# fauzanardh/OsuFusion

Measured on AMD Instinct MI355X. Metric: denoise-steps/sec (train fwd+bwd) at B=32 L=4096, higher is better.
Workload: dtype bf16; 1 GPU; full OsuFusion UNet dim_h=256 (343.5M params) train step: fwd+bwd+grad-norm+clip+AdamW, per-GPU batch 32, L=4096, x (B,6,L), audio (B,96,L) [BASELINE 'audio-ctx=1024x128' maps to the (B,1024,L/8) bottleneck code]; global_batch=32, seq_len=4096, parallelism=dp1

## Files before the change

osufusion_amd/csrc/gemm.hip:

```cpp
#include "common.hpp"
#include <optional>
#include <stdlib.h>

struct RowMap {
  int Lin, Lout, stride, pad, mode;
};
__device__ __forceinline__ int map_row(const RowMap& rm, int i, int t) {
  if (rm.mode == 3) {
    if (t == 3) return (i == rm.Lout - 2) ? rm.Lin - 1 : -1;
    int e = i - t;
    if (e < 0 || (e & 1)) return -1;
    e >>= 1;
    return e < rm.Lin ? e : -1;
  }
  int s = i * rm.stride + t - rm.pad;
  if (rm.mode == 2) {
    if (s < 0 || s >= 2 * rm.Lin) return -1;
    return s >> 1;
  }
  if (rm.mode == 1 && s == rm.Lin) s = rm.Lin - 2;
  return (s >= 0 && s < rm.Lin) ? s : -1;
}

struct GemmArgs {
// ... 1282 lines not shown
          typedef __attribute__((ext_vector_type(8))) short s16x8;
          s16x8 va = {lo[0][0], lo[0][1], lo[0][2], lo[0][3], lo[1][0], lo[1][1], lo[1][2], lo[1][3]};
          s16x8 vb = {hi[0][0], hi[0][1], hi[0][2], hi[0][3], hi[1][0], hi[1][1], hi[1][2], hi[1][3]};
          fa[i] = __builtin_bit_cast(bf16x8, va);
          fb[i] = __builtin_bit_cast(bf16x8, vb);
        }
#pragma unroll
        for (int i = 0; i < 2; ++i)
#pragma unroll
          for (int j = 0; j < 2; ++j)
            acc[i][j] = __builtin_amdgcn_mfma_f32_32x32x16_bf16(fa[i], fb[j], acc[i][j], 0, 0, 0);
      }
    } else if constexpr (SPLIT) {
#pragma unroll
      for (int kk = 0; kk < 2; ++kk) {
        bf16x8 ah[2], al[2], bh[2], bl[2];
#pragma unroll
        for (int i = 0; i < 2; ++i) {
          float xa[8], xb[8];
#pragma unroll
          for (int e = 0; e < 8; ++e) {
            const int row = 16 * kk + 8 * lh + e;
            xa[e] = *reinterpret_cast<const float*>(sy + row * ROWB + (wr * 64 + i * 32 + lr) * 4);
            xb[e] = *reinterpret_cast<const float*>(sx + row * ROWB + (wc * 64 + i * 32 + lr) * 4);
          }
          split_bf16x8(xa, ah[i], al[i]);
          split_bf16x8(xb, bh[i], bl[i]);
        }
#pragma unroll
        for (int i = 0; i < 2; ++i)
#pragma unroll
          for (int j = 0; j < 2; ++j) mfma_x3(acc[i][j], ah[i], al[i], bh[j], bl[j]);
      }
    } else {
#pragma unroll 4
      for (int ks = 0; ks < 16; ++ks) {
        const int row = 2 * ks + lh;
        float fa[2], fb[2];
#pragma unroll
        for (int i = 0; i < 2; ++i) {
          fa[i] = *reinterpret_cast<const float*>(sy + row * ROWB + (wr * 64 + i * 32 + lr) * 4);
          fb[i] = *reinterpret_cast<const float*>(sx + row * ROWB + (wc * 64 + i * 32 + lr) * 4);
        }
#pragma unroll
        for (int i = 0; i < 2; ++i)
#pragma unroll
          for (int j = 0; j < 2; ++j) acc[i][j] = __builtin_amdgcn_mfma_f32_32x32x2f32(fa[i], fb[j], acc[i][j], 0, 0, 0);
      }
    }
  };

  load_regs(m_begin, ry0, rx0);
  if (m_begin + BKM < m_end) load_regs(m_begin + BKM, ry1, rx1);
  store_lds(0, ry0, rx0);
  __syncthreads();
  for (int mb = m_begin; mb < m_end; mb += 2 * BKM) {
    if (mb + 2 * BKM < m_end) load_regs(mb + 2 * BKM, ry0, rx0);
    compute(0);
    if (mb + BKM < m_end) store_lds(1, ry1, rx1);
    __syncthreads();
    if (mb + BKM >= m_end) break;
    if (mb + 3 * BKM < m_end) load_regs(mb + 3 * BKM, ry1, rx1);
    compute(1);
    if (mb + 2 * BKM < m_end) store_lds(0, ry0, rx0);
    __syncthreads();
  }

  float* dW = g.dW + (long)t * g.tapstride;
#pragma unroll
  for (int i = 0; i < 2; ++i)
#pragma unroll
    for (int j = 0; j < 2; ++j) {
      int n2 = n2_0 + wc * 64 + j * 32 + lr;
      if (n2 < g.N2) {
#pragma unroll
        for (int r = 0; r < 16; ++r) {
          int n1 = n1_0 + wr * 64 + i * 32 + (r & 3) + 8 * (r >> 2) + 4 * lh;
          if (n1 < g.N1) atomic_add_f32(dW + (long)n1 * g.ldw + (long)n2 * g.es, acc[i][j][r]);
        }
      }
    }
}

template <bool IL = false>
__device__ __forceinline__ void tn_big_store(const WgradArgs& g, const f32x16 (&acc)[4][2], int split, int t, int n1_0, int n2_0, int wr, int wc,
                                             int lr, int lh) {
  auto n1_of = [&](int i, int r) {
    const int rho = (r & 3) + 8 * (r >> 2) + 4 * lh;
    return n1_0 + wr * 128 + (IL ? 4 * rho + i : i * 32 + rho);
  };
  if (g.ws && g.ws_pk && !IL) {
    uint32_t* out = reinterpret_cast<uint32_t*>(g.ws) + ((long)split * g.taps + t) * (g.N1 >> 1) * g.N2;
#pragma unroll
    for (int i = 0; i < 4; ++i)
#pragma unroll
      for (int j = 0; j < 2; ++j) {
        const int n2 = n2_0 + wc * 64 + j * 32 + lr;
        if (n2 < g.N2) {
#pragma unroll
          for (int r = 0; r < 16; r += 2) {
            const int n1 = n1_of(i, r);
            if (n1 < g.N1) out[(long)(n1 >> 1) * g.N2 + n2] = pack_bf16x2(acc[i][j][r], acc[i][j][r + 1]);
          }
        }
      }
    return;
  }
  if (g.ws) {
    float* out = g.ws + ((long)split * g.taps + t) * g.N1 * g.N2;
#pragma unroll
    for (int i = 0; i < 4; ++i)
#pragma unroll
      for (int j = 0; j < 2; ++j) {
        const int n2 = n2_0 + wc * 64 + j * 32 + lr;
        if (n2 < g.N2) {
#pragma unroll
          for (int r = 0; r < 16; ++r) {
            const int n1 = n1_of(i, r);
            if (n1 < g.N1) out[(long)n1 * g.N2 + n2] = acc[i][j][r];
          }
        }
      }
    return;
  }
  float* dW = g.dW + (long)t * g.tapstride;
#pragma unroll
  for (int i = 0; i < 4; ++i)
#pragma unroll
    for (int j = 0; j < 2; ++j) {
      const int n2 = n2_0 + wc * 64 + j * 32 + lr;
      if (n2 < g.N2) {
#pragma unroll
        for (int r = 0; r < 16; ++r) {
          const int n1 = n1_of(i, r);
          if (n1 < g.N1) atomic_add_f32(dW + (long)n1 * g.ldw + (long)n2 * g.es, acc[i][j][r]);
        }
      }
    }
}

__device__ __forceinline__ float bf16x2_sum(unsigned w, float acc) {
  typedef __attribute__((ext_vector_type(2))) __bf16 bf2;
  return __builtin_amdgcn_fdot2_f32_bf16(__builtin_bit_cast(bf2, w), __builtin_bit_cast(bf2, 0x3F803F80u), acc, false);
}
__device__ __forceinline__ float bf16x8_sum(u32x2 lo, u32x2 hi, float acc) {
  const unsigned w0 = lo.x, w1 = lo.y, w2 = hi.x, w3 = hi.y;
  return bf16x2_sum(w3, bf16x2_sum(w2, bf16x2_sum(w1, bf16x2_sum(w0, acc))));
}

#define OSUF_TR_READ(dst, addr, off) asm volatile("ds_read_b64_tr_b16 %0, %1 offset:%2" : "=v"(dst) : "v"(addr), "n"(off))

__global__ __launch_bounds__(512, 2) void gemm_tn_big_kernel(WgradArgs g) {
  extern __shared__ __attribute__((aligned(16))) char smem[];
  constexpr int BKM = 64, ROWB = 512, TILEB = BKM * ROWB;
  const int tid = threadIdx.x, lane = tid & 63;
  const int wave = __builtin_amdgcn_readfirstlane(tid >> 6);
  const int wr = wave >> 2, wc = wave & 3;
  const int tiles_n2 = (g.N2 + kBig - 1) / kBig;
  const int tiles_n1 = (g.N1 + kBig - 1) / kBig;
  const int ntile = tiles_n1 * tiles_n2;
  const int xcd = blockIdx.x & 7, qid = blockIdx.x >> 3;
  const int unit = xcd * (((int)gridDim.x >> 3) / g.taps) + qid / g.taps;
  const int t = qid % g.taps;
  const int split = unit / ntile, tile = unit % ntile;
  const int n1_0 = (tile / tiles_n2) * kBig, n2_0 = (tile % tiles_n2) * kBig;
  const int m_begin = split * g.rows_per_split;
  const int m_end = min(g.M, m_begin + g.rows_per_split);
  if (m_begin >= m_end) return;
  const bf16_t* dY = reinterpret_cast<const bf16_t*>(g.dY);
  const bf16_t* X = reinterpret_cast<const bf16_t*>(g.X);
  const char* zero = reinterpret_cast<const char*>(g_zero_page);

  int srow[4], scol[4];
#pragma unroll
  for (int i = 0; i < 4; ++i) {
    srow[i] = (wave * 4 + i) * 2 + (lane >> 5);
    scol[i] = ((lane & 31) ^ ((srow[i] & 3) << 2)) * 8;
  }
  int sb_[4], sp_[4];
  const char* py[4];
  bool y_ok[4], x_ok[4];
#pragma unroll
  for (int i = 0; i < 4; ++i) {
    const int m = m_begin + srow[i];
    sb_[i] = m / g.rm.Lout;
    sp_[i] = m - sb_[i] * g.rm.Lout;
    y_ok[i] = n1_0 + scol[i] < g.N1;
    x_ok[i] = n2_0 + scol[i] < g.N2;
    py[i] = reinterpret_cast<const char*>(dY + (long)m * g.ldy + n1_0 + scol[i]);
  }
  const long ystep = (long)BKM * g.ldy * (long)sizeof(bf16_t);
  auto issue = [&](int mb, int buf) {
    char* sy = smem + buf * 2 * TILEB + wave * 4096;
    char* sx = sy + TILEB;
#pragma unroll
    for (int i = 0; i < 4; ++i) {
      const bool in = mb + srow[i] < m_end;
      const char* qy = (in && y_ok[i]) ? py[i] : zero;
      const char* qx = zero;
      if (in && x_ok[i]) {
        const int s2 = map_row(g.rm, sp_[i], t);
        if (s2 >= 0) qx = reinterpret_cast<const char*>(X + (long)(sb_[i] * g.rm.Lin + s2) * g.ldx + n2_0 + scol[i]);
      }
      __builtin_amdgcn_global_load_lds((gas_ptr)qy, (las_ptr)(sy + i * 1024), 16, 0, 0);
      __builtin_amdgcn_global_load_lds((gas_ptr)qx, (las_ptr)(sx + i * 1024), 16, 0, 0);
      py[i] += ystep;
      sp_[i] += BKM;
      while (sp_[i] >= g.rm.Lout) { sp_[i] -= g.rm.Lout; ++sb_[i]; }
    }
  };

  f32x16 acc[4][2];
#pragma unroll
  for (int i = 0; i < 4; ++i)
#pragma unroll
    for (int j = 0; j < 2; ++j)
#pragma unroll
      for (int r = 0; r < 16; ++r) acc[i][j][r] = 0.f;

  const int lr = lane & 31, lh = lane >> 5;
  const int ip = lane & 15, cb = ((lane >> 4) & 1) * 16, tq = ip >> 2, tp = ip & 3;
  uint32_t offA[4], offB[2];
  const uint32_t lds0 = (uint32_t)(uintptr_t)(LDS_PTR(char))smem;
#pragma unroll
  for (int i = 0; i < 4; ++i) offA[i] = (8 * lh + tq) * ROWB + ((((wr * 128 + i * 32 + cb + 4 * tp) * 2)) ^ (tq << 6));
#pragma unroll
  for (int j = 0; j < 2; ++j) offB[j] = TILEB + (8 * lh + tq) * ROWB + ((((wc * 64 + j * 32 + cb + 4 * tp) * 2)) ^ (tq << 6));

  typedef u32x2 frag_half;
  frag_half fa[2][4][2], fb[2][2][2];
#define TN_READS(slot, ks, base)                                                                                   \
  OSUF_TR_READ(fa[slot][0][0], base + offA[0], (ks) * 16 * 512); OSUF_TR_READ(fa[slot][0][1], base + offA[0], ((ks) * 16 + 4) * 512); \
  OSUF_TR_READ(fa[slot][1][0], base + offA[1], (ks) * 16 * 512); OSUF_TR_READ(fa[slot][1][1], base + offA[1], ((ks) * 16 + 4) * 512); \
  OSUF_TR_READ(fa[slot][2][0], base + offA[2], (ks) * 16 * 512); OSUF_TR_READ(fa[slot][2][1], base + offA[2], ((ks) * 16 + 4) * 512); \
  OSUF_TR_READ(fa[slot][3][0], base + offA[3], (ks) * 16 * 512); OSUF_TR_READ(fa[slot][3][1], base + offA[3], ((ks) * 16 + 4) * 512); \
  OSUF_TR_READ(fb[slot][0][0], base + offB[0], (ks) * 16 * 512); OSUF_TR_READ(fb[slot][0][1], base + offB[0], ((ks) * 16 + 4) * 512); \
  OSUF_TR_READ(fb[slot][1][0], base + offB[1], (ks) * 16 * 512); OSUF_TR_READ(fb[slot][1][1], base + offB[1], ((ks) * 16 + 4) * 512);
#define TN_WAIT(slot, n)                                                                                          \
  asm volatile("s_waitcnt lgkmcnt(" #n ")"                                                                        \
               : "+v"(fa[slot][0][0]), "+v"(fa[slot][0][1]), "+v"(fa[slot][1][0]), "+v"(fa[slot][1][1]), "+v"(fa[slot][2][0]),  \
                 "+v"(fa[slot][2][1]), "+v"(fa[slot][3][0]), "+v"(fa[slot][3][1]), "+v"(fb[slot][0][0]), "+v"(fb[slot][0][1]),  \
                 "+v"(fb[slot][1][0]), "+v"(fb[slot][1][1]));                                                     \
  __builtin_amdgcn_sched_barrier(0);
#define TN_MFMA(slot)                                                                                             \
  _Pragma("unroll") for (int i = 0; i < 4; ++i) _Pragma("unroll") for (int j = 0; j < 2; ++j) {                   \
    u32x4 va = {fa[slot][i][0][0], fa[slot][i][0][1], fa[slot][i][1][0], fa[slot][i][1][1]};                       \
    u32x4 vb = {fb[slot][j][0][0], fb[slot][j][0][1], fb[slot][j][1][0], fb[slot][j][1][1]};                       \
    acc[i][j] = __builtin_amdgcn_mfma_f32_32x32x16_bf16(__builtin_bit_cast(bf16x8, va), __builtin_bit_cast(bf16x8, vb), acc[i][j], 0, 0, 0); \
  }

  const bool do_bias = g.dbias != nullptr && n2_0 == 0 && t == 0 && wc == 0;
  float bsum[4] = {0.f, 0.f, 0.f, 0.f};
#define TN_BIAS(slot)                                                                                             \
  if (do_bias) { _Pragma("unroll") for (int i = 0; i < 4; ++i) bsum[i] = bf16x8_sum(fa[slot][i][0], fa[slot][i][1], bsum[i]); }
  issue(m_begin, 0);
  asm volatile("s_waitcnt vmcnt(0)" ::: "memory");
  __builtin_amdgcn_s_barrier();
  int buf = 0;
  for (int mb = m_begin; mb < m_end; mb += BKM, buf ^= 1) {
    const bool more = mb + BKM < m_end;
    if (more) issue(mb + BKM, buf ^ 1);
    const uint32_t base = lds0 + buf * 2 * TILEB;
    TN_READS(0, 0, base)
    TN_READS(1, 1, base)
    TN_WAIT(0, 12)
    TN_MFMA(0)
    TN_BIAS(0)
    TN_READS(0, 2, base)
    TN_WAIT(1, 12)
    TN_MFMA(1)
    TN_BIAS(1)
    TN_READS(1, 3, base)
    TN_WAIT(0, 12)
    TN_MFMA(0)
    TN_BIAS(0)
    TN_WAIT(1, 0)
    TN_MFMA(1)
    TN_BIAS(1)
    asm volatile("s_waitcnt vmcnt(0)" ::: "memory");
    __builtin_amdgcn_s_barrier();
  }
#undef TN_READS
#undef TN_WAIT
#undef TN_MFMA
#undef TN_BIAS
  if (do_bias) {
#pragma unroll
    for (int i = 0; i < 4; ++i) {
      const float v = bsum[i] + __shfl_xor(bsum[i], 32, 64);
      const int n1 = n1_0 + wr * 128 + i * 32 + lr;
      if (lh == 0 && n1 < g.N1) atomic_add_f32(g.dbias + n1, v);
    }
  }

  tn_big_store(g, acc, split, t, n1_0, n2_0, wr, wc, lr, lh);
}

__global__ __launch_bounds__(512, 2) void gemm_tn_big_x3_kernel(WgradArgs g) {
  extern __shared__ __attribute__((aligned(16))) char smem[];
  constexpr int BKM = 32, ROWB = 1024, TILEB = BKM * ROWB;
  const int tid = threadIdx.x, lane = tid & 63;
  const int wave = __builtin_amdgcn_readfirstlane(tid >> 6);
  const int wr = wave >> 2, wc = wave & 3;
  const int tiles_n2 = (g.N2 + kBig - 1) / kBig;
  const int tiles_n1 = (g.N1 + kBig - 1) / kBig;
  const int ntile = tiles_n1 * tiles_n2;
  const int xcd = blockIdx.x & 7, qid = blockIdx.x >> 3;
  const int unit = xcd * (((int)gridDim.x >> 3) / g.taps) + qid / g.taps;
  const int t = qid % g.taps;
  const int split = unit / ntile, tile = unit % ntile;
  const int n1_0 = (tile / tiles_n2) * kBig, n2_0 = (tile % tiles_n2) * kBig;
  const int m_begin = split * g.rows_per_split;
  const int m_end = min(g.M, m_begin + g.rows_per_split);
  if (m_begin >= m_end) return;
  const float* dY = reinterpret_cast<const float*>(g.dY);
  const float* X = reinterpret_cast<const float*>(g.X);
  const char* zero = reinterpret_cast<const char*>(g_zero_page);

  const int scol = lane * 4;
  const bool y_ok = n1_0 + scol < g.N1, x_ok = n2_0 + scol < g.N2;
  int sb_[4], sp_[4];
  const char* py[4];
#pragma unroll
  for (int i = 0; i < 4; ++i) {
    const int m = m_begin + wave * 4 + i;
    sb_[i] = m / g.rm.Lout;
    sp_[i] = m - sb_[i] * g.rm.Lout;
    py[i] = reinterpret_cast<const char*>(dY + (long)m * g.ldy + n1_0 + scol);
  }
  const long ystep = (long)BKM * g.ldy * (long)sizeof(float);
  auto issue = [&](int mb, int buf) {
    char* sy = smem + buf * 2 * TILEB + wave * 4096;
    char* sx = sy + TILEB;
#pragma unroll
    for (int i = 0; i < 4; ++i) {
      const bool in = mb + wave * 4 + i < m_end;
      const char* qy = (in && y_ok) ? py[i] : zero;
      const char* qx = zero;
      if (in && x_ok) {
        const int s2 = map_row(g.rm, sp_[i], t);
        if (s2 >= 0) qx = reinterpret_cast<const char*>(X + (long)(sb_[i] * g.rm.Lin + s2) * g.ldx + n2_0 + scol);
      }
      __builtin_amdgcn_global_load_lds((gas_ptr)qy, (las_ptr)(sy + i * 1024), 16, 0, 0);
      __builtin_amdgcn_global_load_lds((gas_ptr)qx, (las_ptr)(sx + i * 1024), 16, 0, 0);
      py[i] += ystep;
      sp_[i] += BKM;
      while (sp_[i] >= g.rm.Lout) { sp_[i] -= g.rm.Lout; ++sb_[i]; }
    }
  };

  f32x16 acc[4][2];
#pragma unroll
  for (int i = 0; i < 4; ++i)
#pragma unroll
    for (int j = 0; j < 2; ++j)
#pragma unroll
      for (int r = 0; r < 16; ++r) acc[i][j][r] = 0.f;

  const int lr = lane & 31, lh = lane >> 5;
  issue(m_begin, 0);
  asm volatile("s_waitcnt vmcnt(0)" ::: "memory");
  __builtin_amdgcn_s_barrier();
  int buf = 0;
  for (int mb = m_begin; mb < m_end; mb += BKM, buf ^= 1) {
    if (mb + BKM < m_end) issue(mb + BKM, buf ^ 1);
    const char* sy = smem + buf * 2 * TILEB;
    const char* sx = sy + TILEB;
#pragma unroll
    for (int kk = 0; kk < 2; ++kk) {
      bf16x8 ah[4], al[4], bh[2], bl[2];
      {
        f32x4 y[8];
#pragma unroll
        for (int e = 0; e < 8; ++e) y[e] = *reinterpret_cast<const f32x4*>(sy + (16 * kk + 8 * lh + e) * ROWB + (wr * 128 + 4 * lr) * 4);
#pragma unroll
        for (int i = 0; i < 4; ++i) {
          const float x[8] = {y[0][i], y[1][i], y[2][i], y[3][i], y[4][i], y[5][i], y[6][i], y[7][i]};
          split_bf16x8(x, ah[i], al[i]);
        }
      }
#pragma unroll
      for (int j = 0; j < 2; ++j) {
        float x[8];
#pragma unroll
        for (int e = 0; e < 8; ++e) x[e] = *reinterpret_cast<const float*>(sx + (16 * kk + 8 * lh + e) * ROWB + (wc * 64 + j * 32 + lr) * 4);
        split_bf16x8(x, bh[j], bl[j]);
      }
#pragma unroll
      for (int i = 0; i < 4; ++i)
#pragma unroll
        for (int j = 0; j < 2; ++j) mfma_x3(acc[i][j], ah[i], al[i], bh[j], bl[j]);
    }
    asm volatile("s_waitcnt vmcnt(0)" ::: "memory");
    __builtin_amdgcn_s_barrier();
  }
  tn_big_store<true>(g, acc, split, t, n1_0, n2_0, wr, wc, lr, lh);
}

__global__ __launch_bounds__(512, 2) void gemm_tn_taps3_kernel(WgradArgs g) {
  extern __shared__ __attribute__((aligned(16))) char smem[];
  constexpr int BKM = 128, ROWB = 256, YB = BKM * ROWB, XROWS = 132, STAGE = YB + XROWS * ROWB;
  const int tid = threadIdx.x, lane = tid & 63;
  const int wave = __builtin_amdgcn_readfirstlane(tid >> 6);
  const int wr = wave >> 2, wc = wave & 3;
  const int tiles_n2 = (g.N2 + 127) / 128, tiles_n1 = (g.N1 + 127) / 128;
  const int ntile = tiles_n1 * tiles_n2;
  const int xcd = blockIdx.x & 7, local = blockIdx.x >> 3;
  const int unit = xcd * ((int)gridDim.x >> 3) + local;
  const int split = unit / ntile, tile = unit % ntile;
  const int n1_0 = (tile / tiles_n2) * 128, n2_0 = (tile % tiles_n2) * 128;
  const int m_begin = split * g.rows_per_split;
  const int m_end = min(g.M, m_begin + g.rows_per_split);
  if (m_begin >= m_end) return;
  const bf16_t* dY = reinterpret_cast<const bf16_t*>(g.dY);
  const bf16_t* X = reinterpret_cast<const bf16_t*>(g.X);
  const char* zero = reinterpret_cast<const char*>(g_zero_page);
  const int L = g.rm.Lout;

  int yrow[4], prow[5], ycol[4], pcol[5];
#pragma unroll
  for (int i = 0; i < 5; ++i) {
    const int r = ((i < 4 ? wave * 4 + i : 32) * 4) + (lane >> 4);
    const int col = ((lane & 15) ^ ((r & 3) << 2)) * 8;
    prow[i] = r; pcol[i] = col;
    if (i < 4) { yrow[i] = r; ycol[i] = col; }
  }
  int pos = m_begin % L;
  auto issue = [&](int mb, int buf) {
    char* sy = smem + buf * STAGE;
    char* sx = sy + YB;
#pragma unroll
    for (int i = 0; i < 4; ++i) {
      const int m = mb + yrow[i];
      const char* qy = (m < m_end && n1_0 + ycol[i] < g.N1) ? reinterpret_cast<const char*>(dY + (long)m * g.ldy + n1_0 + ycol[i]) : zero;
      __builtin_amdgcn_global_load_lds((gas_ptr)qy, (las_ptr)(sy + (wave * 4 + i) * 1024), 16, 0, 0);
    }
#pragma unroll
    for (int i = 0; i < 5; ++i) {
      if (i == 4 && wave != 0) break;
      const int pr = prow[i];
      const int q = pos - 1 + pr;
      const bool ok = pr < 130 && q >= 0 && q < L && mb - 1 + pr < g.M && n2_0 + pcol[i] < g.N2;
      const char* qx = ok ? reinterpret_cast<const char*>(X + (long)(mb - 1 + pr) * g.ldx + n2_0 + pcol[i]) : zero;
      __builtin_amdgcn_global_load_lds((gas_ptr)qx, (las_ptr)(sx + (i < 4 ? wave * 4 + i : 32) * 1024), 16, 0, 0);
    }
    pos += BKM;
    if (pos >= L) pos -= L;
  };

  f32x16 acc[2][3];
#pragma unroll
  for (int i = 0; i < 2; ++i)
#pragma unroll
    for (int t = 0; t < 3; ++t)
#pragma unroll
      for (int r = 0; r < 16; ++r) acc[i][t][r] = 0.f;

  const int lr = lane & 31, lh = lane >> 5;
  const int ip = lane & 15, cb = ((lane >> 4) & 1) * 16, tq = ip >> 2, tp = ip & 3;
  uint32_t offA[2], offB[3];
  const uint32_t lds0 = (uint32_t)(uintptr_t)(LDS_PTR(char))smem;
#pragma unroll
  for (int i = 0; i < 2; ++i) offA[i] = (8 * lh + tq) * ROWB + (((wr * 64 + i * 32 + cb + 4 * tp) * 2) ^ (tq << 6));
#pragma unroll
  for (int t = 0; t < 3; ++t) offB[t] = YB + (8 * lh + tq + t) * ROWB + (((wc * 32 + cb + 4 * tp) * 2) ^ (((tq + t) & 3) << 6));

  typedef u32x2 frag_half;
  frag_half fa[2][2][2], fb[2][3][2];
#define T3_READS(slot, ks, base)                                                                                   \
  OSUF_TR_READ(fa[slot][0][0], base + offA[0], (ks) * 16 * 256); OSUF_TR_READ(fa[slot][0][1], base + offA[0], ((ks) * 16 + 4) * 256); \
  OSUF_TR_READ(fa[slot][1][0], base + offA[1], (ks) * 16 * 256); OSUF_TR_READ(fa[slot][1][1], base + offA[1], ((ks) * 16 + 4) * 256); \
  OSUF_TR_READ(fb[slot][0][0], base + offB[0], (ks) * 16 * 256); OSUF_TR_READ(fb[slot][0][1], base + offB[0], ((ks) * 16 + 4) * 256); \
  OSUF_TR_READ(fb[slot][1][0], base + offB[1], (ks) * 16 * 256); OSUF_TR_READ(fb[slot][1][1], base + offB[1], ((ks) * 16 + 4) * 256); \
  OSUF_TR_READ(fb[slot][2][0], base + offB[2], (ks) * 16 * 256); OSUF_TR_READ(fb[slot][2][1], base + offB[2], ((ks) * 16 + 4) * 256);
#define T3_WAIT(slot, n)                                                                                          \
  asm volatile("s_waitcnt lgkmcnt(" #n ")"                                                                        \
               : "+v"(fa[slot][0][0]), "+v"(fa[slot][0][1]), "+v"(fa[slot][1][0]), "+v"(fa[slot][1][1]), "+v"(fb[slot][0][0]),  \
                 "+v"(fb[slot][0][1]), "+v"(fb[slot][1][0]), "+v"(fb[slot][1][1]), "+v"(fb[slot][2][0]), "+v"(fb[slot][2][1]));  \
  __builtin_amdgcn_sched_barrier(0);
#define T3_MFMA(slot)                                                                                             \
  _Pragma("unroll") for (int i = 0; i < 2; ++i) _Pragma("unroll") for (int t = 0; t < 3; ++t) {                   \
    u32x4 va = {fa[slot][i][0][0], fa[slot][i][0][1], fa[slot][i][1][0], fa[slot][i][1][1]};                       \
    u32x4 vb = {fb[slot][t][0][0], fb[slot][t][0][1], fb[slot][t][1][0], fb[slot][t][1][1]};                       \
    acc[i][t] = __builtin_amdgcn_mfma_f32_32x32x16_bf16(__builtin_bit_cast(bf16x8, va), __builtin_bit_cast(bf16x8, vb), acc[i][t], 0, 0, 0); \
  }

  const bool do_bias = g.dbias != nullptr && n2_0 == 0 && wc == 0;
  float bsum[2] = {0.f, 0.f};
#define T3_BIAS(slot)                                                                                             \
  if (do_bias) { _Pragma("unroll") for (int i = 0; i < 2; ++i) bsum[i] = bf16x8_sum(fa[slot][i][0], fa[slot][i][1], bsum[i]); }
  issue(m_begin, 0);
  asm volatile("s_waitcnt vmcnt(0)" ::: "memory");
  __builtin_amdgcn_s_barrier();
  int buf = 0;
  for (int mb = m_begin; mb < m_end; mb += BKM, buf ^= 1) {
    if (mb + BKM < m_end) issue(mb + BKM, buf ^ 1);
    const uint32_t base = lds0 + buf * STAGE;
    T3_READS(0, 0, base)
    T3_READS(1, 1, base)
    T3_WAIT(0, 10)  T3_MFMA(0)  T3_BIAS(0)  T3_READS(0, 2, base)
    T3_WAIT(1, 10)  T3_MFMA(1)  T3_BIAS(1)  T3_READS(1, 3, base)
    T3_WAIT(0, 10)  T3_MFMA(0)  T3_BIAS(0)  T3_READS(0, 4, base)
    T3_WAIT(1, 10)  T3_MFMA(1)  T3_BIAS(1)  T3_READS(1, 5, base)
    T3_WAIT(0, 10)  T3_MFMA(0)  T3_BIAS(0)  T3_READS(0, 6, base)
    T3_WAIT(1, 10)  T3_MFMA(1)  T3_BIAS(1)  T3_READS(1, 7, base)
    T3_WAIT(0, 10)  T3_MFMA(0)  T3_BIAS(0)
    T3_WAIT(1, 0)   T3_MFMA(1)  T3_BIAS(1)
    asm volatile("s_waitcnt vmcnt(0)" ::: "memory");
    __builtin_amdgcn_s_barrier();
  }
#undef T3_READS
#undef T3_WAIT
#undef T3_MFMA
#undef T3_BIAS
  if (do_bias) {
#pragma unroll
    for (int i = 0; i < 2; ++i) {
      const float v = bsum[i] + __shfl_xor(bsum[i], 32, 64);
      const int n1 = n1_0 + wr * 64 + i * 32 + lr;
      if (lh == 0 && n1 < g.N1) atomic_add_f32(g.dbias + n1, v);
    }
  }

  if (g.ws && g.ws_pk) {
#pragma unroll
    for (int t = 0; t < 3; ++t) {
      uint32_t* out = reinterpret_cast<uint32_t*>(g.ws) + ((long)split * 3 + t) * (g.N1 >> 1) * g.N2;
#pragma unroll
      for (int i = 0; i < 2; ++i) {
        const int n2 = n2_0 + wc * 32 + lr;
        if (n2 < g.N2) {
#pragma unroll
          for (int r = 0; r < 16; r += 2) {
            const int n1 = n1_0 + wr * 64 + i * 32 + (r & 3) + 8 * (r >> 2) + 4 * lh;
            if (n1 < g.N1) out[(long)(n1 >> 1) * g.N2 + n2] = pack_bf16x2(acc[i][t][r], acc[i][t][r + 1]);
          }
        }
      }
    }
    return;
  }
#pragma unroll
  for (int t = 0; t < 3; ++t) {
    float* out = g.ws ? g.ws + ((long)split * 3 + t) * g.N1 * g.N2 : g.dW + (long)t * g.tapstride;
#pragma unroll
    for (int i = 0; i < 2; ++i) {
      const int n2 = n2_0 + wc * 32 + lr;
      if (n2 < g.N2) {
#pragma unroll
        for (int r = 0; r < 16; ++r) {
          const int n1 = n1_0 + wr * 64 + i * 32 + (r & 3) + 8 * (r >> 2) + 4 * lh;
          if (n1 < g.N1) {
            if (g.ws) out[(long)n1 * g.N2 + n2] = acc[i][t][r];
            else atomic_add_f32(out + (long)n1 * g.ldw + (long)n2 * g.es, acc[i][t][r]);
          }
        }
      }
    }
  }
}

__global__ __launch_bounds__(512, 2) void gemm_tn_taps3_x3_kernel(WgradArgs g) {
  extern __shared__ __attribute__((aligned(16))) char smem[];
  constexpr int BKM = 64, ROWB = 512, YB = BKM * ROWB, XROWS = 66, STAGE = YB + XROWS * ROWB;
  const int tid = threadIdx.x, lane = tid & 63;
  const int wave = __builtin_amdgcn_readfirstlane(tid >> 6);
  const int wr = wave >> 2, wc = wave & 3;
  const int tiles_n2 = (g.N2 + 127) / 128, tiles_n1 = (g.N1 + 127) / 128;
  const int ntile = tiles_n1 * tiles_n2;
  const int xcd = blockIdx.x & 7, local = blockIdx.x >> 3;
  const int unit = xcd * ((int)gridDim.x >> 3) + local;
  const int split = unit / ntile, tile = unit % ntile;
  const int n1_0 = (tile / tiles_n2) * 128, n2_0 = (tile % tiles_n2) * 128;
  const int m_begin = split * g.rows_per_split;
  const int m_end = min(g.M, m_begin + g.rows_per_split);
  if (m_begin >= m_end) return;
  const float* dY = reinterpret_cast<const float*>(g.dY);
  const float* X = reinterpret_cast<const float*>(g.X);
  const char* zero = reinterpret_cast<const char*>(g_zero_page);
  const int L = g.rm.Lout;
  const int col = (lane & 31) * 4;
  const bool y_ok = n1_0 + col < g.N1, x_ok = n2_0 + col < g.N2;
  int pos = m_begin % L;
  auto issue = [&](int mb, int buf) {
    char* sy = smem + buf * STAGE;
    char* sx = sy + YB;
#pragma unroll
    for (int i = 0; i < 4; ++i) {
      const int m = mb + (wave * 4 + i) * 2 + (lane >> 5);
      const char* qy = (m < m_end && y_ok) ? reinterpret_cast<const char*>(dY + (long)m * g.ldy + n1_0 + col) : zero;
      __builtin_amdgcn_global_load_lds((gas_ptr)qy, (las_ptr)(sy + (wave * 4 + i) * 1024), 16, 0, 0);
    }
#pragma unroll
    for (int i = 0; i < 5; ++i) {
      if (i == 4 && wave != 0) break;
      const int gi = i < 4 ? wave * 4 + i : 32;
      const int pr = gi * 2 + (lane >> 5);
      const int q = pos - 1 + pr;
      const bool ok = q >= 0 && q < L && mb - 1 + pr < g.M && x_ok;
      const char* qx = ok ? reinterpret_cast<const char*>(X + (long)(mb - 1 + pr) * g.ldx + n2_0 + col) : zero;
      __builtin_amdgcn_global_load_lds((gas_ptr)qx, (las_ptr)(sx + gi * 1024), 16, 0, 0);
    }
    pos += BKM;
    if (pos >= L) pos -= L;
  };

  f32x16 acc[2][3];
#pragma unroll
  for (int i = 0; i < 2; ++i)
#pragma unroll
    for (int t = 0; t < 3; ++t)
#pragma unroll
      for (int r = 0; r < 16; ++r) acc[i][t][r] = 0.f;

  const int lr = lane & 31, lh = lane >> 5;
  issue(m_begin, 0);
  asm volatile("s_waitcnt vmcnt(0)" ::: "memory");
  __builtin_amdgcn_s_barrier();
  int buf = 0;
  for (int mb = m_begin; mb < m_end; mb += BKM, buf ^= 1) {
    if (mb + BKM < m_end) issue(mb + BKM, buf ^ 1);
    const char* sy = smem + buf * STAGE;
    const char* sx = sy + YB;
#pragma unroll
    for (int kk = 0; kk < 4; ++kk) {
      bf16x8 ah[2], al[2], bh[3], bl[3];
      {
        typedef __attribute__((ext_vector_type(2))) float f32x2;
        f32x2 y[8];
#pragma unroll
        for (int e = 0; e < 8; ++e) y[e] = *reinterpret_cast<const f32x2*>(sy + (16 * kk + 8 * lh + e) * ROWB + (wr * 64 + 2 * lr) * 4);
#pragma unroll
        for (int i = 0; i < 2; ++i) {
          const float x[8] = {y[0][i], y[1][i], y[2][i], y[3][i], y[4][i], y[5][i], y[6][i], y[7][i]};
          split_bf16x8(x, ah[i], al[i]);
        }
      }
      {
        float xw[10];
#pragma unroll
        for (int e = 0; e < 10; ++e) xw[e] = *reinterpret_cast<const float*>(sx + (16 * kk + 8 * lh + e) * ROWB + (wc * 32 + lr) * 4);
#pragma unroll
        for (int t = 0; t < 3; ++t) {
          const float x[8] = {xw[t], xw[t + 1], xw[t + 2], xw[t + 3], xw[t + 4], xw[t + 5], xw[t + 6], xw[t + 7]};
          split_bf16x8(x, bh[t], bl[t]);
        }
      }
#pragma unroll
      for (int i = 0; i < 2; ++i)
#pragma unroll
        for (int t = 0; t < 3; ++t) mfma_x3(acc[i][t], ah[i], al[i], bh[t], bl[t]);
    }
    asm volatile("s_waitcnt vmcnt(0)" ::: "memory");
    __builtin_amdgcn_s_barrier();
  }
#pragma unroll
  for (int t = 0; t < 3; ++t) {
    float* out = g.ws ? g.ws + ((long)split * 3 + t) * g.N1 * g.N2 : g.dW + (long)t * g.tapstride;
#pragma unroll
    for (int i = 0; i < 2; ++i) {
      const int n2 = n2_0 + wc * 32 + lr;
      if (n2 < g.N2) {
#pragma unroll
// ... 366 lines not shown
  g.A = A; g.W = W; g.C = C; g.C2 = C2; g.R = R; g.U = U; g.bias = bias; g.rscale = rscale; g.stats = stats;
  g.delta = delta; g.heads = heads;
  g.lda = lda; g.ldw = ldw; g.tapstride = tapstride; g.ldc = ldc; g.ldc2 = ldc2; g.ldr = ldr; g.ldu = ldu;
  g.M = M; g.N = N; g.K = K; g.taps = taps;
  g.rm = RowMap{Lin, Lout, stride, pad, mode};
  g.act = act;
  const int grid = ((M + kTile - 1) / kTile) * ((N + kTile - 1) / kTile);
  const int lds = 2 * kStageBytes + 512;
  static bool attr_done = false;
  if (!attr_done) {
    (void)hipFuncSetAttribute((const void*)gemm_nt_glds_kernel<bf16_t>, hipFuncAttributeMaxDynamicSharedMemorySize, lds);
    (void)hipFuncSetAttribute((const void*)gemm_nt_glds_kernel<float>, hipFuncAttributeMaxDynamicSharedMemorySize, lds);
    (void)hipFuncSetAttribute((const void*)(gemm_nt_glds_kernel<float, true>), hipFuncAttributeMaxDynamicSharedMemorySize, lds);
    attr_done = true;
  }
  if (dtype == OSUF_DT_BF16 && N <= 32 && N % 8 == 0 && ldc % 8 == 0 && M >= 4096 && !C2 && !R && !U && !bias && !rscale && !stats &&
      act == 0) {
    const int lds_sk = 2 * kSkStage;
    static bool sk_attr = ((void)hipFuncSetAttribute((const void*)gemm_nt_skinny_kernel, hipFuncAttributeMaxDynamicSharedMemorySize, lds_sk), true);
    (void)sk_attr;
    hipLaunchKernelGGL(gemm_nt_skinny_kernel, dim3((M + kBig - 1) / kBig), dim3(512), lds_sk, stream, g);
    return osuf_launch_status();
  }
  const std::optional<long> bigenv = big_min_tiles_override();
  const long min_tiles = bigenv.value_or(192);
  const long big_tiles = (long)((M + kBig - 1) / kBig) * ((N + kBig - 1) / kBig);
  const bool use_big = (dtype == OSUF_DT_BF16 || dtype == OSUF_DT_F32X3) && min_tiles > 0 && big_tiles >= min_tiles && (N >= 192 || bigenv) && N % 8 == 0 &&
                       ldc % 8 == 0 && (!C2 || ldc2 % 8 == 0) && (!R || ldr % 8 == 0) && (!U || ldu % 8 == 0) &&
                       (!bias || (reinterpret_cast<uintptr_t>(bias) & 31) == 0) && (!rscale || (reinterpret_cast<uintptr_t>(rscale) & 31) == 0);
  if (use_big) {
    const int lds_big = 2 * kBigStage + 2112;
    const int lds_p8 = kP8Tbl + taps * kBig * 4;
    static bool big_attr = false;
    if (!big_attr) {
      (void)hipFuncSetAttribute((const void*)gemm_nt_big_kernel<bf16_t>, hipFuncAttributeMaxDynamicSharedMemorySize, lds_big);
      (void)hipFuncSetAttribute((const void*)(gemm_nt_big_kernel<float, true>), hipFuncAttributeMaxDynamicSharedMemorySize, lds_big);
      big_attr = true;
    }
    const long tm = (M + kBig - 1) / kBig, tn = (N + kBig - 1) / kBig;
    const dim3 grid_big((int)(((tm + 7) / 8) * 8 * tn));
    const bool halo3 = taps == 3 && mode == 0 && stride == 1 && pad == 1 && Lin == Lout && Lout % kBig == 0 && K % (dtype == OSUF_DT_BF16 ? 64 : 32) == 0 &&
                       getenv("OSUF_GEMM_NOHALO") == nullptr;
    if (halo3) {
      static bool halo_attr = ((void)hipFuncSetAttribute((const void*)gemm_nt_big_halo3_kernel<bf16_t>, hipFuncAttributeMaxDynamicSharedMemorySize, lds_big),
                               (void)hipFuncSetAttribute((const void*)gemm_nt_big_halo3_kernel<float>, hipFuncAttributeMaxDynamicSharedMemorySize, lds_big), true);
      (void)halo_attr;
      if (dtype == OSUF_DT_BF16 && getenv("OSUF_GEMM_NO8P") == nullptr && K <= 8192) {
        const int lds_h8 = kH8B + 65536 + 2112;
        static bool h8_attr = ((void)hipFuncSetAttribute((const void*)gemm_nt_big8_halo3_kernel, hipFuncAttributeMaxDynamicSharedMemorySize, lds_h8), true);
        (void)h8_attr;
        hipLaunchKernelGGL(gemm_nt_big8_halo3_kernel, grid_big, dim3(512), lds_h8, stream, g);
      } else if (dtype == OSUF_DT_BF16) hipLaunchKernelGGL(gemm_nt_big_halo3_kernel<bf16_t>, grid_big, dim3(512), lds_big, stream, g);
      else hipLaunchKernelGGL(gemm_nt_big_halo3_kernel<float>, grid_big, dim3(512), lds_big, stream, g);
    } else if (dtype == OSUF_DT_BF16 && getenv("OSUF_GEMM_NO8P") == nullptr && taps <= kP8MaxTaps && K <= 8192 && K % 64 == 0) {
      const int lds_p8_max = kP8Tbl + kP8MaxTaps * kBig * 4;
      static bool p8_attr = ((void)hipFuncSetAttribute((const void*)gemm_nt_big8_kernel, hipFuncAttributeMaxDynamicSharedMemorySize, lds_p8_max), true);
      (void)p8_attr;
      hipLaunchKernelGGL(gemm_nt_big8_kernel, grid_big, dim3(512), lds_p8, stream, g);
    } else if (dtype == OSUF_DT_F32X3) hipLaunchKernelGGL((gemm_nt_big_kernel<float, true>), grid_big, dim3(512), lds_big, stream, g);
    else hipLaunchKernelGGL(gemm_nt_big_kernel<bf16_t>, grid_big, dim3(512), lds_big, stream, g);
  } else {
    if (dtype == OSUF_DT_BF16) hipLaunchKernelGGL(gemm_nt_glds_kernel<bf16_t>, dim3(grid), dim3(256), lds, stream, g);
    else if (dtype == OSUF_DT_F32X3) hipLaunchKernelGGL((gemm_nt_glds_kernel<float, true>), dim3(grid), dim3(256), lds, stream, g);
    else hipLaunchKernelGGL(gemm_nt_glds_kernel<float>, dim3(grid), dim3(256), lds, stream, g);
  }
  return osuf_launch_status();
}

static bool tn_big_plan(int dtype, int M, int N1, int N2, int taps, int* rows_out, int* splits_out) {
  const std::optional<long> bigenv = big_min_tiles_override();
  const bool forced = bigenv == 1, off = bigenv && *bigenv <= 0;
  if ((dtype != OSUF_DT_BF16 && dtype != OSUF_DT_F32X3) || off || !(forced || (N1 >= 64 && N2 >= 64 && (N1 >= 192 || N2 >= 192)))) return false;
  const int btiles = ((N1 + kBig - 1) / kBig) * ((N2 + kBig - 1) / kBig);
  int sp = (256 + btiles * taps / 2) / (btiles * taps);
  if (sp < 1) sp = 1;
  while (sp > 1 && ((sp * btiles + 7) / 8) * 8 * taps > 256) --sp;
  int rows = (M + sp - 1) / sp;
  rows = ((rows + 63) / 64) * 64;
  if (rows_out) *rows_out = rows;
  if (splits_out) *splits_out = (M + rows - 1) / rows;
  return true;
}

extern "C" long osuf_gemm_tn_workspace_bytes(int dtype, int M, int N1, int N2, int taps) {
  int rows, sp;
  if (M <= 0 || N1 <= 0 || N2 <= 0 || taps <= 0 || !tn_big_plan(dtype, M, N1, N2, taps, &rows, &sp)) return 0;
  if ((N1 * (long)N2 * taps) % 4) return 0;
  return (long)sp * taps * N1 * N2 * (long)sizeof(float);
}
static bool wgrad_pk(int dtype, int N1, int N2) {
  return dtype == OSUF_DT_BF16 && (N1 % 2) == 0 && (N2 % 4) == 0 && getenv("OSUF_WGRAD_F32_PARTIALS") == nullptr;
}

extern "C" int osuf_colsum(int dtype, const void* Y, long ldy, int M, int N, float* out, hipStream_t stream);

static int gemm_tn_launch(int dtype, const void* dY, long ldy, const void* X, long ldx, float* dW, long ldw, long tapstride,
                          int M, int N1, int N2, int taps, int Lin, int Lout, int stride, int pad, int mode,
                          int splits, int out_layout, int accumulate, float* workspace, long workspace_bytes, float* dbias, hipStream_t stream) {
  long es = 1;
  if (out_layout == 1) { ldw = (long)N2 * taps; tapstride = 1; es = taps; }
  else if (out_layout != 0) return OSUF_EINVAL;
  const int epc = dtype == OSUF_DT_BF16 ? 8 : 4;
  if (dtype != OSUF_DT_BF16 && dtype != OSUF_DT_F32 && dtype != OSUF_DT_F32X3) return OSUF_EUNSUPPORTED;
  if (M <= 0 || N1 <= 0 || N2 <= 0 || taps <= 0 || Lout <= 0 || Lin <= 0 || M % Lout) return OSUF_EINVAL;
  if (N1 % epc || N2 % epc || ldy % epc || ldx % epc) return OSUF_EINVAL;
  if (!aligned16(dY) || !aligned16(X)) return OSUF_EINVAL;
  auto bias_by_colsum = [&]() -> int {
    return dbias ? osuf_colsum(dtype == OSUF_DT_BF16 ? OSUF_DT_BF16 : OSUF_DT_F32, dY, ldy, M, N1, dbias, stream) : OSUF_OK;
  };
  const int bkm = dtype == OSUF_DT_BF16 ? 64 : 32;
  if (splits <= 0 && dtype == OSUF_DT_BF16 && N2 <= 32 && M >= 4096) {
    WgradArgs gs{};
    gs.dY = dY; gs.X = X; gs.dW = dW; gs.ws = nullptr; gs.es = es; gs.ldy = ldy; gs.ldx = ldx; gs.ldw = ldw; gs.tapstride = tapstride;
    gs.M = M; gs.N1 = N1; gs.N2 = N2; gs.taps = taps; gs.rm = RowMap{Lin, Lout, stride, pad, mode};
    const int tiles_n1 = (N1 + kBig - 1) / kBig;
    int sp = 512 / (tiles_n1 * taps);
    if (sp < 1) sp = 1;
    int rows = (M + sp - 1) / sp;
    rows = ((rows + 63) / 64) * 64;
    if (rows < 256) rows = 256;
    sp = (M + rows - 1) / rows;
    gs.rows_per_split = rows;
    if (!accumulate) {
      if (out_layout == 0 && !(ldw == N2 && (taps == 1 || tapstride == (long)N1 * N2))) return OSUF_EINVAL;
      (void)hipMemsetAsync(dW, 0, (size_t)taps * N1 * N2 * sizeof(float), stream);
    }
    const int lds_sk = 2 * (64 * 512 + 64 * 64);
    static bool sk_attr = ((void)hipFuncSetAttribute((const void*)gemm_tn_skinny_kernel, hipFuncAttributeMaxDynamicSharedMemorySize, lds_sk), true);
    (void)sk_attr;
    hipLaunchKernelGGL(gemm_tn_skinny_kernel, dim3(tiles_n1 * taps * sp), dim3(512), lds_sk, stream, gs);
    if (int rc = bias_by_colsum()) return rc;
    return osuf_launch_status();
  }
  if (splits <= 0 && (dtype == OSUF_DT_BF16 || dtype == OSUF_DT_F32X3) && taps == 3 && mode == 0 && stride == 1 && pad == 1 && Lin == Lout && Lout % 128 == 0 && N1 >= 64 &&
      N2 >= 64 && tn_big_plan(dtype, M, N1, N2, taps, nullptr, nullptr) && getenv("OSUF_GEMM_NOHALO") == nullptr) {
    const int btiles = ((N1 + 127) / 128) * ((N2 + 127) / 128);
    int sp = 256 / btiles;
    if (sp < 1) sp = 1;
    int rows = (M + sp - 1) / sp;
    rows = ((rows + 127) / 128) * 128;
    sp = (M + rows - 1) / rows;
    WgradArgs gb{};
    gb.dY = dY; gb.X = X; gb.dW = dW; gb.ldy = ldy; gb.ldx = ldx; gb.ldw = ldw; gb.tapstride = tapstride;
    gb.M = M; gb.N1 = N1; gb.N2 = N2; gb.taps = taps; gb.rm = RowMap{Lin, Lout, stride, pad, mode};
    gb.rows_per_split = rows;
    const long n = (long)taps * N1 * N2;
    const bool dense = (out_layout == 1 && ((long)N1 * N2) % 4 == 0) || (out_layout == 0 && ldw == N2 && tapstride == (long)N1 * N2 && n % 4 == 0 && aligned16(dW));
    gb.ws = (workspace && dense && aligned16(workspace) && workspace_bytes >= (long)sp * n * (long)sizeof(float)) ? workspace : nullptr;
    gb.es = es;
    gb.ws_pk = gb.ws && wgrad_pk(dtype, N1, N2);
    gb.dbias = dtype == OSUF_DT_BF16 ? dbias : nullptr;
    if (dtype != OSUF_DT_BF16) { if (int rc = bias_by_colsum()) return rc; }
    if (!gb.ws && !accumulate) (void)hipMemsetAsync(dW, 0, (size_t)n * sizeof(float), stream);
    const int lds_t3 = 2 * (128 * 256 + 132 * 256);
    static bool t3_attr = ((void)hipFuncSetAttribute((const void*)gemm_tn_taps3_kernel, hipFuncAttributeMaxDynamicSharedMemorySize, lds_t3),
                           (void)hipFuncSetAttribute((const void*)gemm_tn_taps3_x3_kernel, hipFuncAttributeMaxDynamicSharedMemorySize, lds_t3), true);
    (void)t3_attr;
    const dim3 grid_t3(((sp * btiles + 7) / 8) * 8);
    if (dtype == OSUF_DT_F32X3) hipLaunchKernelGGL(gemm_tn_taps3_x3_kernel, grid_t3, dim3(512), lds_t3, stream, gb);
    else hipLaunchKernelGGL(gemm_tn_taps3_kernel, grid_t3, dim3(512), lds_t3, stream, gb);
    if (gb.ws) launch_wgrad_reduce(gb, dW, N1, N2, taps, sp, out_layout, accumulate, true, stream);
    return osuf_launch_status();
  }
  {
    int rows, sp;
    if (splits <= 0 && tn_big_plan(dtype, M, N1, N2, taps, &rows, &sp)) {
      WgradArgs gb{};
      gb.dY = dY; gb.X = X; gb.dW = dW; gb.ldy = ldy; gb.ldx = ldx; gb.ldw = ldw; gb.tapstride = tapstride;
      gb.M = M; gb.N1 = N1; gb.N2 = N2; gb.taps = taps; gb.rm = RowMap{Lin, Lout, stride, pad, mode};
      gb.rows_per_split = rows;
      const long n = (long)taps * N1 * N2;
      const bool dense = (out_layout == 1 && ((long)N1 * N2) % 4 == 0) || (out_layout == 0 && ldw == N2 && (taps == 1 || tapstride == (long)N1 * N2) && n % 4 == 0 && aligned16(dW));
      gb.ws = (workspace && dense && aligned16(workspace) && workspace_bytes >= (long)sp * n * (long)sizeof(float)) ? workspace : nullptr;
      gb.es = es;
      gb.ws_pk = gb.ws && wgrad_pk(dtype, N1, N2);
      gb.dbias = dtype == OSUF_DT_BF16 ? dbias : nullptr;
      if (dtype != OSUF_DT_BF16) { if (int rc = bias_by_colsum()) return rc; }
      if (!gb.ws && !accumulate) (void)hipMemsetAsync(dW, 0, (size_t)n * sizeof(float), stream);
      const int btiles = ((N1 + kBig - 1) / kBig) * ((N2 + kBig - 1) / kBig);
      const int lds_big = 2 * 65536;
      static bool attr = false;
      if (!attr) {
        (void)hipFuncSetAttribute((const void*)gemm_tn_big_kernel, hipFuncAttributeMaxDynamicSharedMemorySize, lds_big);
        (void)hipFuncSetAttribute((const void*)gemm_tn_big_x3_kernel, hipFuncAttributeMaxDynamicSharedMemorySize, lds_big);
        attr = true;
      }
      if (dtype == OSUF_DT_F32X3) hipLaunchKernelGGL(gemm_tn_big_x3_kernel, dim3(((sp * btiles + 7) / 8) * 8 * taps), dim3(512), lds_big, stream, gb);
      else hipLaunchKernelGGL(gemm_tn_big_kernel, dim3(((sp * btiles + 7) / 8) * 8 * taps), dim3(512), lds_big, stream, gb);
      if (gb.ws) launch_wgrad_reduce(gb, dW, N1, N2, taps, sp, out_layout, accumulate, out_layout == 0 || taps == 3, stream);
      return osuf_launch_status();
    }
  }
  const int tiles = ((N1 + kTile - 1) / kTile) * ((N2 + kTile - 1) / kTile);
  if (splits <= 0) {
    splits = (768 + tiles * taps - 1) / (tiles * taps);
  }
  int rows = (M + splits - 1) / splits;
  rows = ((rows + bkm - 1) / bkm) * bkm;
  splits = (M + rows - 1) / rows;
  WgradArgs g{};
  g.dY = dY; g.X = X; g.dW = dW; g.ldy = ldy; g.ldx = ldx; g.ldw = ldw; g.tapstride = tapstride;
  g.M = M; g.N1 = N1; g.N2 = N2; g.taps = taps; g.rm = RowMap{Lin, Lout, stride, pad, mode};
  g.rows_per_split = rows;
  g.ws = nullptr;
  g.es = es;
  if (!accumulate) {
    if (out_layout == 0 && !(ldw == N2 && (taps == 1 || tapstride == (long)N1 * N2))) return OSUF_EINVAL;
    (void)hipMemsetAsync(dW, 0, (size_t)taps * N1 * N2 * sizeof(float), stream);
  }
  if (int rc = bias_by_colsum()) return rc;
  const int lds = 4 * 16384;
  if (dtype == OSUF_DT_BF16) {
    hipLaunchKernelGGL(gemm_tn_kernel<bf16_t>, dim3(tiles, taps, splits), dim3(256), lds, stream, g);
  } else if (dtype == OSUF_DT_F32X3) {
    hipLaunchKernelGGL((gemm_tn_kernel<float, true>), dim3(tiles, taps, splits), dim3(256), lds, stream, g);
  } else {
    hipLaunchKernelGGL(gemm_tn_kernel<float>, dim3(tiles, taps, splits), dim3(256), lds, stream, g);
  }
  return osuf_launch_status();
}

extern "C" int osuf_gemm_tn(int dtype, const void* dY, long ldy, const void* X, long ldx, float* dW, long ldw, long tapstride,
                            int M, int N1, int N2, int taps, int Lin, int Lout, int stride, int pad, int mode,
                            int splits, int out_layout, int accumulate, float* workspace, long workspace_bytes, hipStream_t stream) {
  return gemm_tn_launch(dtype, dY, ldy, X, ldx, dW, ldw, tapstride, M, N1, N2, taps, Lin, Lout, stride, pad, mode, splits, out_layout, accumulate,
                        workspace, workspace_bytes, nullptr, stream);
}

extern "C" int osuf_gemm_tn_bias(int dtype, const void* dY, long ldy, const void* X, long ldx, float* dW, long ldw, long tapstride,
                                 int M, int N1, int N2, int taps, int Lin, int Lout, int stride, int pad, int mode,
                                 int splits, int out_layout, int accumulate, float* workspace, long workspace_bytes, float* dbias,
                                 hipStream_t stream) {
  if (!dbias) return OSUF_EINVAL;
  return gemm_tn_launch(dtype, dY, ldy, X, ldx, dW, ldw, tapstride, M, N1, N2, taps, Lin, Lout, stride, pad, mode, splits, out_layout, accumulate,
                        workspace, workspace_bytes, dbias, stream);
}

extern "C" int osuf_colsum(int dtype, const void* Y, long ldy, int M, int N, float* out, hipStream_t stream) {
  if (M <= 0 || N <= 0 || N % 8 || ldy % 8 || !aligned16(Y)) return OSUF_EINVAL;
  const int rows_per_block = 256;
  dim3 grid((N + 255) / 256, (M + rows_per_block - 1) / rows_per_block);
  if (dtype == OSUF_DT_BF16) {
    hipLaunchKernelGGL(colsum_kernel<bf16_t>, grid, dim3(256), 0, stream, (const bf16_t*)Y, ldy, M, N, out, rows_per_block);
  } else if (dtype == OSUF_DT_F32) {
    hipLaunchKernelGGL(colsum_kernel<float>, grid, dim3(256), 0, stream, (const float*)Y, ldy, M, N, out, rows_per_block);
  } else {
    return OSUF_EUNSUPPORTED;
  }
  return osuf_launch_status();
}
```

Baseline: 5.592 steps/s.

## Deepen wgrad GEMM pipelines to four-stage LDS ring with smaller K steps

```diff
diff --git a/osufusion_amd/csrc/gemm.hip b/osufusion_amd/csrc/gemm.hip
--- a/osufusion_amd/csrc/gemm.hip
+++ b/osufusion_amd/csrc/gemm.hip
@@ -1458,7 +1458,7 @@
 
 __global__ __launch_bounds__(512, 2) void gemm_tn_big_kernel(WgradArgs g) {
   extern __shared__ __attribute__((aligned(16))) char smem[];
-  constexpr int BKM = 64, ROWB = 512, TILEB = BKM * ROWB;
+  constexpr int BKM = 32, ROWB = 512, TILEB = BKM * ROWB, SLOT = 2 * TILEB;
   const int tid = threadIdx.x, lane = tid & 63;
   const int wave = __builtin_amdgcn_readfirstlane(tid >> 6);
   const int wr = wave >> 2, wc = wave & 3;
@@ -1477,17 +1477,17 @@
   const bf16_t* X = reinterpret_cast<const bf16_t*>(g.X);
   const char* zero = reinterpret_cast<const char*>(g_zero_page);
 
-  int srow[4], scol[4];
-#pragma unroll
-  for (int i = 0; i < 4; ++i) {
-    srow[i] = (wave * 4 + i) * 2 + (lane >> 5);
+  int srow[2], scol[2];
+#pragma unroll
+  for (int i = 0; i < 2; ++i) {
+    srow[i] = (wave * 2 + i) * 2 + (lane >> 5);
     scol[i] = ((lane & 31) ^ ((srow[i] & 3) << 2)) * 8;
   }
-  int sb_[4], sp_[4];
-  const char* py[4];
-  bool y_ok[4], x_ok[4];
-#pragma unroll
-  for (int i = 0; i < 4; ++i) {
+  int sb_[2], sp_[2];
+  const char* py[2];
+  bool y_ok[2], x_ok[2];
+#pragma unroll
+  for (int i = 0; i < 2; ++i) {
     const int m = m_begin + srow[i];
     sb_[i] = m / g.rm.Lout;
     sp_[i] = m - sb_[i] * g.rm.Lout;
@@ -1496,11 +1496,13 @@
     py[i] = reinterpret_cast<const char*>(dY + (long)m * g.ldy + n1_0 + scol[i]);
   }
   const long ystep = (long)BKM * g.ldy * (long)sizeof(bf16_t);
-  auto issue = [&](int mb, int buf) {
-    char* sy = smem + buf * 2 * TILEB + wave * 4096;
+  const int nst = (m_end - m_begin + BKM - 1) / BKM;
+  auto issue = [&](int j) {
+    const int mb = m_begin + j * BKM;
+    char* sy = smem + (j & 3) * SLOT + wave * 2048;
     char* sx = sy + TILEB;
 #pragma unroll
-    for (int i = 0; i < 4; ++i) {
+    for (int i = 0; i < 2; ++i) {
       const bool in = mb + srow[i] < m_end;
       const char* qy = (in && y_ok[i]) ? py[i] : zero;
       const char* qx = zero;
@@ -1559,33 +1561,43 @@
   float bsum[4] = {0.f, 0.f, 0.f, 0.f};
 #define TN_BIAS(slot)                                                                                             \
   if (do_bias) { _Pragma("unroll") for (int i = 0; i < 4; ++i) bsum[i] = bf16x8_sum(fa[slot][i][0], fa[slot][i][1], bsum[i]); }
-  issue(m_begin, 0);
-  asm volatile("s_waitcnt vmcnt(0)" ::: "memory");
-  __builtin_amdgcn_s_barrier();
-  int buf = 0;
-  for (int mb = m_begin; mb < m_end; mb += BKM, buf ^= 1) {
-    const bool more = mb + BKM < m_end;
-    if (more) issue(mb + BKM, buf ^ 1);
-    const uint32_t base = lds0 + buf * 2 * TILEB;
-    TN_READS(0, 0, base)
+  auto stage = [&](int j, auto kind) {
+    constexpr int KIND = decltype(kind)::value;
+    const uint32_t base = lds0 + (j & 3) * SLOT, next = lds0 + ((j + 1) & 3) * SLOT;
     TN_READS(1, 1, base)
     TN_WAIT(0, 12)
     TN_MFMA(0)
     TN_BIAS(0)
-    TN_READS(0, 2, base)
-    TN_WAIT(1, 12)
+    __builtin_amdgcn_sched_barrier(0);
+    if constexpr (KIND == 0) {
+      asm volatile("s_waitcnt vmcnt(4)" ::: "memory");
+      __builtin_amdgcn_s_barrier();
+      if (j + 3 < nst) issue(j + 3);
+    } else if constexpr (KIND == 1) {
+      asm volatile("s_waitcnt vmcnt(0)" ::: "memory");
+      __builtin_amdgcn_s_barrier();
+    }
+    if constexpr (KIND != 2) {
+      TN_READS(0, 0, next)
+      TN_WAIT(1, 12)
+    } else {
+      TN_WAIT(1, 0)
+    }
     TN_MFMA(1)
     TN_BIAS(1)
-    TN_READS(1, 3, base)
-    TN_WAIT(0, 12)
-    TN_MFMA(0)
-    TN_BIAS(0)
-    TN_WAIT(1, 0)
-    TN_MFMA(1)
-    TN_BIAS(1)
-    asm volatile("s_waitcnt vmcnt(0)" ::: "memory");
-    __builtin_amdgcn_s_barrier();
-  }
+  };
+  issue(0);
+  if (nst > 1) issue(1);
+  if (nst > 2) issue(2);
+  if (nst > 2) asm volatile("s_waitcnt vmcnt(8)" ::: "memory");
+  else if (nst > 1) asm volatile("s_waitcnt vmcnt(4)" ::: "memory");
+  else asm volatile("s_waitcnt vmcnt(0)" ::: "memory");
+  __builtin_amdgcn_s_barrier();
+  TN_READS(0, 0, lds0)
+  int j = 0;
+  for (; j + 2 < nst; ++j) stage(j, IntC<0>{});
+  if (j + 1 < nst) { stage(j, IntC<1>{}); ++j; }
+  stage(j, IntC<2>{});
 #undef TN_READS
 #undef TN_WAIT
 #undef TN_MFMA
@@ -1705,7 +1717,7 @@
 
 __global__ __launch_bounds__(512, 2) void gemm_tn_taps3_kernel(WgradArgs g) {
   extern __shared__ __attribute__((aligned(16))) char smem[];
-  constexpr int BKM = 128, ROWB = 256, YB = BKM * ROWB, XROWS = 132, STAGE = YB + XROWS * ROWB;
+  constexpr int BKM = 64, ROWB = 256, YB = BKM * ROWB, XROWS = 68, STAGE = YB + XROWS * ROWB;
   const int tid = threadIdx.x, lane = tid & 63;
   const int wave = __builtin_amdgcn_readfirstlane(tid >> 6);
   const int wr = wave >> 2, wc = wave & 3;
@@ -1723,32 +1735,34 @@
   const char* zero = reinterpret_cast<const char*>(g_zero_page);
   const int L = g.rm.Lout;
 
-  int yrow[4], prow[5], ycol[4], pcol[5];
-#pragma unroll
-  for (int i = 0; i < 5; ++i) {
-    const int r = ((i < 4 ? wave * 4 + i : 32) * 4) + (lane >> 4);
+  int yrow[2], prow[3], ycol[2], pcol[3];
+#pragma unroll
+  for (int i = 0; i < 3; ++i) {
+    const int r = ((i < 2 ? wave * 2 + i : 16) * 4) + (lane >> 4);
     const int col = ((lane & 15) ^ ((r & 3) << 2)) * 8;
     prow[i] = r; pcol[i] = col;
-    if (i < 4) { yrow[i] = r; ycol[i] = col; }
+    if (i < 2) { yrow[i] = r; ycol[i] = col; }
   }
   int pos = m_begin % L;
-  auto issue = [&](int mb, int buf) {
-    char* sy = smem + buf * STAGE;
+  const int nst = (m_end - m_begin + BKM - 1) / BKM;
+  auto issue = [&](int j) {
+    const int mb = m_begin + j * BKM;
+    char* sy = smem + (j & 3) * STAGE;
     char* sx = sy + YB;
 #pragma unroll
-    for (int i = 0; i < 4; ++i) {
+    for (int i = 0; i < 2; ++i) {
       const int m = mb + yrow[i];
       const char* qy = (m < m_end && n1_0 + ycol[i] < g.N1) ? reinterpret_cast<const char*>(dY + (long)m * g.ldy + n1_0 + ycol[i]) : zero;
-      __builtin_amdgcn_global_load_lds((gas_ptr)qy, (las_ptr)(sy + (wave * 4 + i) * 1024), 16, 0, 0);
-    }
-#pragma unroll
-    for (int i = 0; i < 5; ++i) {
-      if (i == 4 && wave != 0) break;
+      __builtin_amdgcn_global_load_lds((gas_ptr)qy, (las_ptr)(sy + (wave * 2 + i) * 1024), 16, 0, 0);
+    }
+#pragma unroll
+    for (int i = 0; i < 3; ++i) {
+      if (i == 2 && wave != 0) break;
       const int pr = prow[i];
       const int q = pos - 1 + pr;
-      const bool ok = pr < 130 && q >= 0 && q < L && mb - 1 + pr < g.M && n2_0 + pcol[i] < g.N2;
+      const bool ok = pr < 66 && q >= 0 && q < L && mb - 1 + pr < g.M && n2_0 + pcol[i] < g.N2;
       const char* qx = ok ? reinterpret_cast<const char*>(X + (long)(mb - 1 + pr) * g.ldx + n2_0 + pcol[i]) : zero;
-      __builtin_amdgcn_global_load_lds((gas_ptr)qx, (las_ptr)(sx + (i < 4 ? wave * 4 + i : 32) * 1024), 16, 0, 0);
+      __builtin_amdgcn_global_load_lds((gas_ptr)qx, (las_ptr)(sx + (i < 2 ? wave * 2 + i : 16) * 1024), 16, 0, 0);
     }
     pos += BKM;
     if (pos >= L) pos -= L;
@@ -1795,26 +1809,46 @@
   float bsum[2] = {0.f, 0.f};
 #define T3_BIAS(slot)                                                                                             \
   if (do_bias) { _Pragma("unroll") for (int i = 0; i < 2; ++i) bsum[i] = bf16x8_sum(fa[slot][i][0], fa[slot][i][1], bsum[i]); }
-  issue(m_begin, 0);
-  asm volatile("s_waitcnt vmcnt(0)" ::: "memory");
-  __builtin_amdgcn_s_barrier();
-  int buf = 0;
-  for (int mb = m_begin; mb < m_end; mb += BKM, buf ^= 1) {
-    if (mb + BKM < m_end) issue(mb + BKM, buf ^ 1);
-    const uint32_t base = lds0 + buf * STAGE;
-    T3_READS(0, 0, base)
+#define T3_VMWAIT(n)                                                                                              \
+  if (wave == 0) asm volatile("s_waitcnt vmcnt(%0)" ::"n"(5 * (n)) : "memory");                                    \
+  else asm volatile("s_waitcnt vmcnt(%0)" ::"n"(4 * (n)) : "memory");
+  auto stage = [&](int j, auto kind) {
+    constexpr int KIND = decltype(kind)::value;
+    const uint32_t base = lds0 + (j & 3) * STAGE, next = lds0 + ((j + 1) & 3) * STAGE;
     T3_READS(1, 1, base)
     T3_WAIT(0, 10)  T3_MFMA(0)  T3_BIAS(0)  T3_READS(0, 2, base)
     T3_WAIT(1, 10)  T3_MFMA(1)  T3_BIAS(1)  T3_READS(1, 3, base)
-    T3_WAIT(0, 10)  T3_MFMA(0)  T3_BIAS(0)  T3_READS(0, 4, base)
-    T3_WAIT(1, 10)  T3_MFMA(1)  T3_BIAS(1)  T3_READS(1, 5, base)
-    T3_WAIT(0, 10)  T3_MFMA(0)  T3_BIAS(0)  T3_READS(0, 6, base)
-    T3_WAIT(1, 10)  T3_MFMA(1)  T3_BIAS(1)  T3_READS(1, 7, base)
     T3_WAIT(0, 10)  T3_MFMA(0)  T3_BIAS(0)
-    T3_WAIT(1, 0)   T3_MFMA(1)  T3_BIAS(1)
-    asm volatile("s_waitcnt vmcnt(0)" ::: "memory");
-    __builtin_amdgcn_s_barrier();
-  }
+    __builtin_amdgcn_sched_barrier(0);
+    if constexpr (KIND == 0) {
+      T3_VMWAIT(1)
+      __builtin_amdgcn_s_barrier();
+      if (j + 3 < nst) issue(j + 3);
+    } else if constexpr (KIND == 1) {
+      T3_VMWAIT(0)
+      __builtin_amdgcn_s_barrier();
+    }
+    if constexpr (KIND != 2) {
+      T3_READS(0, 0, next)
+      T3_WAIT(1, 10)
+    } else {
+      T3_WAIT(1, 0)
+    }
+    T3_MFMA(1)  T3_BIAS(1)
+  };
+  issue(0);
+  if (nst > 1) issue(1);
+  if (nst > 2) issue(2);
+  if (nst > 2) { T3_VMWAIT(2) }
+  else if (nst > 1) { T3_VMWAIT(1) }
+  else { T3_VMWAIT(0) }
+  __builtin_amdgcn_s_barrier();
+  T3_READS(0, 0, lds0)
+  int j = 0;
+  for (; j + 2 < nst; ++j) stage(j, IntC<0>{});
+  if (j + 1 < nst) { stage(j, IntC<1>{}); ++j; }
+  stage(j, IntC<2>{});
+#undef T3_VMWAIT
 #undef T3_READS
 #undef T3_WAIT
 #undef T3_MFMA
@@ -2487,12 +2521,12 @@
     gb.dbias = dtype == OSUF_DT_BF16 ? dbias : nullptr;
     if (dtype != OSUF_DT_BF16) { if (int rc = bias_by_colsum()) return rc; }
     if (!gb.ws && !accumulate) (void)hipMemsetAsync(dW, 0, (size_t)n * sizeof(float), stream);
-    const int lds_t3 = 2 * (128 * 256 + 132 * 256);
+    const int lds_t3 = 4 * (64 * 256 + 68 * 256), lds_t3_x3 = 2 * (128 * 256 + 132 * 256);
     static bool t3_attr = ((void)hipFuncSetAttribute((const void*)gemm_tn_taps3_kernel, hipFuncAttributeMaxDynamicSharedMemorySize, lds_t3),
-                           (void)hipFuncSetAttribute((const void*)gemm_tn_taps3_x3_kernel, hipFuncAttributeMaxDynamicSharedMemorySize, lds_t3), true);
+                           (void)hipFuncSetAttribute((const void*)gemm_tn_taps3_x3_kernel, hipFuncAttributeMaxDynamicSharedMemorySize, lds_t3_x3), true);
     (void)t3_attr;
     const dim3 grid_t3(((sp * btiles + 7) / 8) * 8);
-    if (dtype == OSUF_DT_F32X3) hipLaunchKernelGGL(gemm_tn_taps3_x3_kernel, grid_t3, dim3(512), lds_t3, stream, gb);
+    if (dtype == OSUF_DT_F32X3) hipLaunchKernelGGL(gemm_tn_taps3_x3_kernel, grid_t3, dim3(512), lds_t3_x3, stream, gb);
     else hipLaunchKernelGGL(gemm_tn_taps3_kernel, grid_t3, dim3(512), lds_t3, stream, gb);
     if (gb.ws) launch_wgrad_reduce(gb, dW, N1, N2, taps, sp, out_layout, accumulate, true, stream);
     return osuf_launch_status();
```

Result: no change. 5.599 steps/s (median of 6 runs) (+0.1%).
